# ruotianluo/ImageCaptioning.pytorch

Measured on NVIDIA H100. Metric: captions/sec at beam=5 seq_len=20, higher is better.
Workload: dtype f32 (fp32-grade: split-fp16 x3 tensor-core passes, fp32 accumulate)

## Files before the change

### imagecaptioning.pytorch_b200/_lib.py

```python
from __future__ import annotations

import ctypes
import os
from ctypes import POINTER, Structure, c_char_p, c_double, c_float, c_int, c_long, c_longlong, c_ulonglong, c_void_p

PKG = os.path.dirname(os.path.abspath(__file__))
LIB_PATH = os.path.join(PKG, 'libcapb200.so')

MODE_SIMT_FP32, MODE_TC_F16X3, MODE_TC_F16X1 = 0, 1, 2
MODES = {'simt_fp32': MODE_SIMT_FP32, 'tc_f16x3': MODE_TC_F16X3, 'tc_f16x1': MODE_TC_F16X1}
OP_MODES = dict(MODES, skinny_tf32x3=3, skinny_fp32=4, tf32x3_tc=5, tf32x3_tc_dgrad=6, tf32x3_tc_wgrad=7)
FAMILY_UPDOWN, FAMILY_NEWFC, FAMILY_ATT2IN2 = 0, 1, 2
FAMILY_AOA = 3
ENSEMBLE_MAX_MEMBERS = 8
SAMPLE_GREEDY, SAMPLE_MULTINOMIAL, SAMPLE_FORCED, SAMPLE_TEACHER, SAMPLE_TOPK, SAMPLE_TOPP = 0, 1, 2, 3, 4, 5


class ModelCfg(Structure):
    _fields_ = [('family', c_int), ('vocab_size', c_int), ('input_encoding_size', c_int), ('rnn_size', c_int), ('att_hid_size', c_int),
                ('fc_feat_size', c_int), ('att_feat_size', c_int), ('seq_length', c_int), ('numeric_mode', c_int)]


WEIGHT_FIELDS = ['embed', 'fc_embed_w', 'fc_embed_b', 'att_embed_w', 'att_embed_b', 'ctx2att_w', 'ctx2att_b', 'logit_w', 'logit_b',
                 'att_lstm_w_ih', 'att_lstm_w_hh', 'att_lstm_b_ih', 'att_lstm_b_hh', 'lang_lstm_w_ih', 'lang_lstm_w_hh', 'lang_lstm_b_ih',
# ... 162 lines not shown
                                        'logit_b')]


class GemmEpilogue(Structure):
    _fields_ = [('bias', c_void_p), ('row_bias', c_void_p), ('ld_row_bias', c_long), ('rows_per_group', c_int), ('residual', c_void_p),
                ('ld_res', c_long), ('relu', c_int), ('C', c_void_p), ('ldc', c_long), ('C_hi', c_void_p), ('C_lo', c_void_p), ('ldcs', c_long),
                ('lstm', c_int), ('H', c_int), ('c_prev', c_void_p), ('ld_cprev', c_long), ('src_row', c_void_p), ('c_out', c_void_p),
                ('ld_cout', c_long), ('gather_bias', c_void_p), ('ld_gb', c_long), ('gather_idx', c_void_p), ('h_f', c_void_p), ('h_hi', c_void_p),
                ('h_lo', c_void_p), ('ld_h', c_long)]


SIGNATURES = {
    'capb200_last_error': (c_char_p, []),
    'capb200_abi_version': (c_int, []),
    'capb200_range_status': (c_int, [c_int]),
    'capb200_linear': (c_int, [c_void_p, c_long, c_void_p, c_long, c_void_p, c_void_p, c_long, c_int, c_int, c_int, c_int, c_int, c_void_p]),
    'capb200_bench_linear': (c_int, [c_void_p, c_void_p, c_void_p, c_void_p, c_int, c_int, c_int, c_int, c_int, c_void_p, c_void_p]),
    'capb200_gemm_tile_n': (c_int, [c_int, c_int]),
    'capb200_gemm_tile_m': (c_int, [c_int, c_int]),
    'capb200_lstm_cell': (c_int, [c_void_p, c_int, c_void_p, c_void_p, c_void_p, c_void_p, c_void_p, c_void_p, c_void_p, c_void_p, c_int, c_int,
                                  c_int, c_void_p]),
    'capb200_additive_attention': (c_int, [c_void_p, c_void_p, c_void_p, c_void_p, c_void_p, c_void_p, c_void_p, c_int, c_int, c_int, c_int, c_int,
                                           c_void_p]),
    'capb200_log_softmax_topk': (c_int, [c_void_p, c_long, c_int, c_int, c_int, c_int, c_void_p, c_void_p, c_void_p]),
    'capb200_vocab_stats_topk': (c_int, [c_void_p, c_long, c_int, c_int, c_int, c_int, c_void_p, c_void_p, c_void_p, c_void_p]),
    'capb200_vocab_select': (c_int, [c_void_p, c_long, c_int, c_int, c_int, c_float, c_float, c_ulonglong, c_ulonglong, c_void_p, c_int, c_void_p,
                                     c_void_p, c_void_p]),
    'capb200_engine_create': (c_void_p, [POINTER(ModelCfg)]),
    'capb200_engine_destroy': (None, [c_void_p]),
    'capb200_engine_bind_weights': (c_int, [c_void_p, POINTER(Weights), c_void_p]),
    'capb200_engine_set_logit_layers': (c_int, [c_void_p, c_int]),
    'capb200_engine_bind_logit_head': (c_int, [c_void_p, POINTER(c_void_p), POINTER(c_void_p), c_void_p]),
    'capb200_engine_bind_logit_head_grads': (c_int, [c_void_p, POINTER(c_void_p), POINTER(c_void_p)]),
    'capb200_engine_set_logit_dropout': (c_int, [c_void_p, c_float]),
    'capb200_decode_beam': (c_int, [c_void_p, c_void_p, c_void_p, c_void_p, c_int, c_int, POINTER(BeamOpts), c_void_p, c_void_p, c_void_p, c_void_p,
                                    c_void_p, c_void_p, c_void_p]),
    'capb200_decode_beam_form': (c_int, [c_int, c_void_p, c_void_p, c_void_p, c_void_p, c_int, c_int, POINTER(BeamOpts), c_void_p, c_void_p, c_void_p,
                                         c_void_p, c_void_p, c_void_p, c_void_p]),
    'capb200_beam_record_logprobs': (c_int, [c_void_p, c_int, c_int, c_void_p, c_void_p]),
    'capb200_decode_beam_diverse': (c_int, [c_void_p, c_void_p, c_void_p, c_void_p, c_int, c_int, POINTER(DiverseOpts), c_void_p, c_void_p, c_void_p,
                                            c_void_p, c_void_p, c_void_p, c_void_p]),
    'capb200_decode_sample': (c_int, [c_void_p, c_void_p, c_void_p, c_void_p, c_int, c_int, POINTER(SampleOpts), c_void_p, c_long, c_void_p, c_void_p,
                                      c_void_p, c_void_p]),
    'capb200_engine_launch_count': (c_long, [c_void_p]),
    'capb200_engine_set_profiling': (c_int, [c_void_p, c_int]),
    'capb200_engine_read_profile': (c_int, [c_void_p, c_int, c_void_p, c_void_p, c_void_p, c_int]),
# ... 159 lines not shown
```

### imagecaptioning.pytorch_b200/csrc/engine.cu

```cuda
#include <map>
#include <mutex>
#include <vector>

#include "../../include/capb200.h"
#include "common.cuh"
#include "kernels.cuh"
#include "engine_common.cuh"
#include "train_common.cuh"

namespace capb200 {

static thread_local std::string g_last_error;
void set_error(const std::string& msg) { g_last_error = msg; }
const char* last_error_cstr() { return g_last_error.c_str(); }

__global__ void capb_fill_int_kernel(int* p, int n, int v) {
    const int i = blockIdx.x * blockDim.x + threadIdx.x;
    if (i < n) p[i] = v;
}
__global__ void capb_load_token_column_kernel(const long long* src, long ld, int col, int n, int* dst) {
    const int i = blockIdx.x * blockDim.x + threadIdx.x;
    if (i < n) dst[i] = (int)src[(long)i * ld + col];
}
__global__ void capb_store_token_column_kernel(const int* src, int n, long long* dst, long ld, int col) {
// ... 277 lines not shown
                g.epi.lstm = 1; g.epi.H = H;
                g.epi.c_prev = e->c0[cur]; g.epi.ld_cprev = e->ld_c; g.epi.src_row = src_row;
                g.epi.c_out = e->c0[nxt]; g.epi.ld_cout = e->ld_c;
                g.epi.gather_bias = xg ? e->xgate : nullptr; g.epi.ld_gb = e->ld_xgate; g.epi.gather_idx = tokens;
                g.epi.h_f = e->h0_out.v.f; g.epi.h_hi = e->h0_out.v.hi; g.epi.h_lo = e->h0_out.v.lo; g.epi.ld_h = e->h0_out.v.ld;
            } else {
                g.epi.C = e->gates.v.f; g.epi.ldc = e->gates.v.ld;
            }
            if (run_gemm(e, G_LSTM1, g, e->capRows, st)) return 1;
        }
        if (!e->tc) {
            e->launches++;
            if (lstm_pointwise_launch(rows, H, e->gates.v.f, e->gates.v.ld, src_row, e->c0[cur], e->ld_c, e->c0[nxt], e->ld_c, e->h0_out.v,
                                      xg ? e->xgate : nullptr, e->ld_xgate, tokens, st)) return 1;
        }
        {
            GemmProblem g;
            g.M = rows; g.N = A; g.nseg = 1;
            g.seg[0] = seg_of(e->h0_out.v, w.h2att_w, H, e->p_h2att, H);
            g.epi.bias = w.h2att_b;
            g.epi.C = e->att_h.v.f; g.epi.ldc = e->att_h.v.ld;
            if (run_gemm(e, G_H2ATT, g, e->capRows, st)) return 1;
        }
        e->launches += 2;
        if (additive_attention_launch(n_images, rpi, R, A, H, e->att_h.v.f, e->att_h.v.ld, e->p_att.v.f, e->p_att.v.ld, e->att_e.v.f, e->att_e.v.ld,
                                      mask, R, w.alpha_w, w.alpha_b, e->att_score, e->att_res.v, st)) return 1;
        {
            GemmProblem g;
            g.M = rows; g.N = 4 * H; g.nseg = 3;
            g.seg[0] = seg_of(e->att_res.v, w.lang_lstm_w_ih, 2 * H, e->p_l_ih_a, H);
            g.seg[1] = seg_of(e->h0_out.v, w.lang_lstm_w_ih + H, 2 * H, e->p_l_ih_h, H);
            g.seg[2] = seg_of(e->h1_in.v, w.lang_lstm_w_hh, H, e->p_l_hh, H);
            if (e->tc) {
                g.epi.bias = e->bsum_lang_il;
                g.epi.lstm = 1; g.epi.H = H;
                g.epi.c_prev = e->c1[cur]; g.epi.ld_cprev = e->ld_c; g.epi.src_row = src_row;
                g.epi.c_out = e->c1[nxt]; g.epi.ld_cout = e->ld_c;
                g.epi.h_f = e->h1_out.v.f; g.epi.h_hi = e->h1_out.v.hi; g.epi.h_lo = e->h1_out.v.lo; g.epi.ld_h = e->h1_out.v.ld;
            } else {
                g.epi.bias = e->bsum_lang;
                g.epi.C = e->gates.v.f; g.epi.ldc = e->gates.v.ld;
            }
            if (run_gemm(e, G_LSTM2, g, e->capRows, st)) return 1;
        }
        if (!e->tc) {
            e->launches++;
            if (lstm_pointwise_launch(rows, H, e->gates.v.f, e->gates.v.ld, src_row, e->c1[cur], e->ld_c, e->c1[nxt], e->ld_c, e->h1_out.v,
                                      nullptr, 0, nullptr, st)) return 1;
        }
        e->core_cur = nxt;
        return logit_gemm(e, e->h1_out.v, rows, logits, ld_logits, st);
    }
    if (e->cfg.family == CAPB200_FAMILY_ATT2IN2) {
        StateCopy s0, s1;
        s0.src = e->h0_out.v.f; s0.ld_src = e->h0_out.v.ld; s0.dst = e->h0_in.v;
        e->launches++;
        if (state_gather_embed_launch(rows, tokens, src_row, w.embed, E, E, 1, e->xt.v, H, 1, s0, s1, st)) return 1;
        const int cur = e->core_cur, nxt = cur ^ 1;
        {
            GemmProblem g;
            g.M = rows; g.N = A; g.nseg = 1;
            g.seg[0] = seg_of(e->h0_in.v, w.h2att_w, H, e->p_h2att, H);
            g.epi.bias = w.h2att_b;
            g.epi.C = e->att_h.v.f; g.epi.ldc = e->att_h.v.ld;
            if (run_gemm(e, G_H2ATT, g, e->capRows, st)) return 1;
        }
        e->launches += 2;
        if (additive_attention_launch(n_images, rpi, R, A, H, e->att_h.v.f, e->att_h.v.ld, e->p_att.v.f, e->p_att.v.ld, e->att_e.v.f, e->att_e.v.ld,
                                      mask, R, w.alpha_w, w.alpha_b, e->att_score, e->att_res.v, st)) return 1;
        {
            GemmProblem g;
            g.M = rows; g.N = 5 * H; g.nseg = 2;
            g.seg[0] = seg_of(e->xt.v, w.i2h_w, E, e->p_i2h, E);
            g.seg[1] = seg_of(e->h0_in.v, w.h2h_w, H, e->p_h2h, H);
            g.epi.bias = e->bsum_core;
            g.epi.C = e->gates.v.f; g.epi.ldc = e->gates.v.ld;
            if (run_gemm(e, G_CORE, g, e->capRows, st)) return 1;
        }
        {
            GemmProblem g;
            g.M = rows; g.N = 2 * H; g.nseg = 1;
            g.seg[0] = seg_of(e->att_res.v, w.a2c_w, H, e->p_a2c, H);
            g.epi.residual = e->gates.v.f + 3 * H; g.epi.ld_res = e->gates.v.ld;
            g.epi.C = e->gates.v.f + 3 * H; g.epi.ldc = e->gates.v.ld;
            if (run_gemm(e, G_A2C, g, e->capRows, st)) return 1;
        }
        e->launches++;
        if (maxout_pointwise_launch(rows, H, e->gates.v.f, e->gates.v.ld, src_row, e->c0[cur], e->ld_c, e->c0[nxt], e->ld_c, e->h0_out.v, st)) return 1;
        e->core_cur = nxt;
        return logit_gemm(e, e->h0_out.v, rows, logits, ld_logits, st);
// ... 459 lines not shown
                      const float* b_hh, float* h_out, float* c_out, int M, int H, int mode, void* stream) {
    cudaStream_t st = static_cast<cudaStream_t>(stream);
    CAPB_REQUIRE(x && h && c && w_ih && w_hh && b_ih && b_hh && h_out && c_out, "null argument");
    float* gates = nullptr;
    CAPB_CHECK_CUDA(cudaMallocAsync(&gates, sizeof(float) * ((size_t)M * 4 * H + 4 * H), st));
    float* bsum = gates + (size_t)M * 4 * H;
    add_vec_kernel<<<cdiv(4 * H, 256), 256, 0, st>>>(b_ih, b_hh, bsum, 4 * H);
    int rc = capb200_linear(x, Kx, w_ih, Kx, bsum, gates, 4 * H, M, 4 * H, Kx, 0, mode, stream);
    float* g2 = nullptr;
    if (!rc) {
        CAPB_CHECK_CUDA(cudaMallocAsync(&g2, sizeof(float) * (size_t)M * 4 * H, st));
        rc = capb200_linear(h, H, w_hh, H, nullptr, g2, 4 * H, M, 4 * H, H, 0, mode, stream);
        if (!rc) add_vec_kernel<<<cdiv(M * 4 * H, 256), 256, 0, st>>>(gates, g2, gates, M * 4 * H);
    }
    if (!rc) {
        ActView ho; ho.f = h_out; ho.ld = H;
        rc = lstm_pointwise_launch(M, H, gates, 4 * H, nullptr, c, H, c_out, H, ho, nullptr, 0, nullptr, st);
    }
    if (g2) cudaFreeAsync(g2, st);
    cudaFreeAsync(gates, st);
    return rc;
}

int capb200_additive_attention(const float* att_h, const float* p_att, const float* att, const float* mask, const float* alpha_w,
                               const float* alpha_b, float* out, int n_images, int rows_per_image, int R, int A, int H, void* stream) {
    CAPB_REQUIRE(att_h && p_att && att && alpha_w && alpha_b && out, "null argument");
    ActView o; o.f = out; o.ld = H;
    cudaStream_t st = static_cast<cudaStream_t>(stream);
    float* scratch = nullptr;
    CAPB_CHECK_CUDA(cudaMallocAsync(&scratch, sizeof(float) * (size_t)n_images * rows_per_image * R, st));
    const int rc = additive_attention_launch(n_images, rows_per_image, R, A, H, att_h, A, p_att, A, att, H, mask, R, alpha_w, alpha_b, scratch, o, st);
    cudaFreeAsync(scratch, st);
    return rc;
}

int capb200_log_softmax_topk(float* logits, long ld, int rows, int V1, int twice, int k, float* top_val, int* top_idx, void* stream) {
    CAPB_REQUIRE(logits != nullptr && rows > 0 && V1 > 0, "bad argument");
    VocabStepArgs va;
    va.rows = rows; va.V1 = V1; va.logits = logits; va.ld = ld; va.twice = twice; va.topk = k; va.top_val = top_val; va.top_idx = top_idx;
    return vocab_step_launch(va, static_cast<cudaStream_t>(stream));
}

int capb200_vocab_stats_topk(const float* logits, long ld, int rows, int V1, int twice, int k, float* stats, float* top_val, int* top_idx, void* stream) {
    CAPB_REQUIRE(logits != nullptr && stats != nullptr && top_val != nullptr && top_idx != nullptr, "null argument");
    CAPB_REQUIRE(rows > 0 && V1 > 0 && ld >= V1 && k > 0, "bad argument");
    CAPB_REQUIRE((reinterpret_cast<uintptr_t>(stats) & 7) == 0, "stats must be 8-byte aligned");
    VocabStepArgs va;
    va.rows = rows; va.V1 = V1; va.logits = const_cast<float*>(logits); va.ld = ld; va.twice = twice;
    va.topk = k; va.top_val = top_val; va.top_idx = top_idx;
    va.stats = reinterpret_cast<float2*>(stats);
    return vocab_step_launch(va, static_cast<cudaStream_t>(stream));
}

int capb200_vocab_select(float* logits, long ld, int rows, int V1, int select, float top, float temperature, unsigned long long seed,
                         unsigned long long step, int* unfinished, int first_step, int* tokens_out, float* picked_lp, void* stream) {
    CAPB_REQUIRE(logits != nullptr && tokens_out != nullptr && picked_lp != nullptr, "null argument");
// ... 745 lines not shown
```

### imagecaptioning.pytorch_b200/csrc/kernels.cuh

```cuda
#pragma once
#include "common.cuh"

namespace capb200 {

struct ActView {
    float* f = nullptr;
    __half* hi = nullptr;
    __half* lo = nullptr;
    long ld = 0;
};

struct StateCopy {
    const float* src = nullptr;
    long ld_src = 0;
    ActView dst;
};

__device__ __forceinline__ void copy_states4(long r, int src, int c4, int nstate, const StateCopy& sc0, const StateCopy& sc1) {
    float4 v0 = make_float4(0.f, 0.f, 0.f, 0.f), v1 = v0;
    if (src >= 0) {
        v0 = *reinterpret_cast<const float4*>(sc0.src + (long)src * sc0.ld_src + 4 * c4);
        if (nstate > 1) v1 = *reinterpret_cast<const float4*>(sc1.src + (long)src * sc1.ld_src + 4 * c4);
    }
    for (int s = 0; s < nstate; ++s) {
// ... 2 lines not shown
        *reinterpret_cast<float4*>(o.f + r * o.ld + 4 * c4) = v;
        if (o.hi != nullptr) {
            __align__(8) __half h[4];
            __align__(8) __half l[4];
            split_f32(v.x, h[0], l[0]); split_f32(v.y, h[1], l[1]); split_f32(v.z, h[2], l[2]); split_f32(v.w, h[3], l[3]);
            *reinterpret_cast<uint2*>(o.hi + r * o.ld + 4 * c4) = *reinterpret_cast<const uint2*>(h);
            *reinterpret_cast<uint2*>(o.lo + r * o.ld + 4 * c4) = *reinterpret_cast<const uint2*>(l);
        }
    }
}

int state_gather_embed_launch(int rows, const int* tokens, const int* src_row, const float* emb, long ld_emb, int E, int relu,
                              ActView xt, int H, int nstate, StateCopy sc0, StateCopy sc1, cudaStream_t stream);
int lstm_pointwise_launch(int rows, int H, const float* gates, long ld_g, const int* src_row, const float* c_prev, long ld_cp,
                          float* c_out, long ld_co, ActView h_out, const float* gather_bias, long ld_gb, const int* gather_idx,
                          cudaStream_t stream);
int relu_copy_launch(const float* x, long n, ActView out_flat, cudaStream_t stream);
int lstm_ln_launch(int rows, int H, const float* gates, long ld_g, const float* c_prev, long ld_cp, float* c_out, long ld_co, float* h_out, long ld_h,
                   const float* ln_a, const float* ln_b, float eps, float* ln_out, long ld_ln, cudaStream_t stream);
int maxout_pointwise_launch(int rows, int H, const float* sums, long ld_s, const int* src_row, const float* c_prev, long ld_cp,
                            float* c_out, long ld_co, ActView h_out, cudaStream_t stream);
int additive_attention_launch(int n_images, int rpi, int R, int A, int H, const float* att_h, long ld_ah, const float* p_att, long ld_pa,
                              const float* att, long ld_at, const float* mask, long ld_mask, const float* alpha_w, const float* alpha_b,
                              float* score_scratch , ActView out, cudaStream_t stream, float* alpha_out = nullptr );
int mask_rows_launch(ActView x, int n_images, int R, int cols, const float* mask, long ld_mask, cudaStream_t stream);
int ss_select_launch(int rows, int V1, const float* prev_logp, long ld, const long long* labels, long ld_labels, int col, unsigned long long seed, float prob,
                     int* tok_out, cudaStream_t stream);

struct DecodeEdits {
    int constraint = 0;
    int unk_col = -1;
    int n_bad = 0;
    const int* bad = nullptr;
    int trigrams = 0;
    int trigram_rows = 0;
    __host__ __device__ bool any() const { return constraint != 0 || unk_col >= 0 || n_bad > 0 || trigrams != 0; }
    __host__ __device__ int kinds() const { return (constraint ? 1 : 0) + (unk_col >= 0 ? 1 : 0) + (n_bad > 0 ? 1 : 0); }
};

struct VocabStepArgs {
    int rows = 0;
    int V1 = 0;
    float* logits = nullptr;
    long ld = 0;
    int twice = 0;
    float2* stats = nullptr;
    int topk = 0;
// ... 221 lines not shown
```

### imagecaptioning.pytorch_b200/csrc/pointwise.cu

```cuda
#include "common.cuh"
#include "kernels.cuh"

namespace capb200 {

static int pw_blocks(long total) {
    long b = (total + 255) / 256;
    return (int)(b > sm_count() * 8 ? sm_count() * 8 : b);
}

namespace {

__device__ __forceinline__ float sigmoidf_(float x) { return fast_sigmoid(x); }

__device__ __forceinline__ void store_act(const ActView& o, long row, int col, float v) {
    o.f[row * o.ld + col] = v;
    if (o.hi != nullptr) {
        __half h, l;
        split_f32(v, h, l);
        o.hi[row * o.ld + col] = h;
        o.lo[row * o.ld + col] = l;
    }
}

__global__ void state_gather_embed_kernel(int rows, const int* __restrict__ tokens, const int* __restrict__ src_row,
// ... 84 lines not shown
#pragma unroll
    for (int u = 0; u < 8; ++u) { const int c = threadIdx.x + 256 * u; if (c < H) ln_out[(long)r * ld_ln + c] = __ldg(ln_a + c) * (hv[u] - mean) * inv + __ldg(ln_b + c); }
}

__global__ void maxout_pointwise_kernel(int rows, int H, const float* __restrict__ sums, long ld_s, const int* __restrict__ src_row,
                                        const float* __restrict__ c_prev, long ld_cp, float* __restrict__ c_out, long ld_co, ActView h_out) {
    const long total = (long)rows * H;
    for (long i = blockIdx.x * (long)blockDim.x + threadIdx.x; i < total; i += (long)gridDim.x * blockDim.x) {
        const int r = (int)(i / H), c = (int)(i % H);
        const float* s = sums + (long)r * ld_s;
        const float gi = sigmoidf_(s[c]), gf = sigmoidf_(s[H + c]), go = sigmoidf_(s[2 * H + c]);
        const float gg = fmaxf(s[3 * H + c], s[4 * H + c]);
        const int src = src_row ? src_row[r] : r;
        const float cp = (src < 0 || c_prev == nullptr) ? 0.f : c_prev[(long)src * ld_cp + c];
        const float cn = gf * cp + gi * gg;
        const float hn = go * fast_tanh(cn);
        c_out[(long)r * ld_co + c] = cn;
        store_act(h_out, r, c, hn);
    }
}

constexpr int ATT_JB = 5;
constexpr int ATT_SW = 8;
template <int NA>
__global__ void __launch_bounds__(ATT_SW * 32, NA <= 16 ? 5 : 2) att_score_kernel(int rpi, int R, int A, const float* __restrict__ att_h, long ld_ah,
                                                                const float* __restrict__ p_att, long ld_pa, const float* __restrict__ alpha_w,
                                                                const float* __restrict__ alpha_b_ptr, float* __restrict__ score) {
    extern __shared__ float s_ah[];
    constexpr int AP = NA * 32;
    float* s_w = s_ah + ATT_JB * AP;
    constexpr float kC = 2.885390081777927f;
    const int img = blockIdx.y;
    const int warp = threadIdx.x >> 5, lane = threadIdx.x & 31;
    const int r = blockIdx.x * ATT_SW + warp;
    const float alpha_b = __ldg(alpha_b_ptr);
    float pv[NA];
    const bool live = r < R;
    const float* pr = p_att + ((long)img * R + (live ? r : 0)) * ld_pa;
    for (int i = threadIdx.x; i < AP; i += ATT_SW * 32) s_w[i] = (i < A) ? __ldg(alpha_w + i) : 0.f;
    __syncthreads();
    float wsum = 0.f;
#pragma unroll
    for (int k = 0; k < NA; ++k) {
        const int a = (NA % 4 == 0) ? 128 * (k >> 2) + 4 * lane + (k & 3) : lane + 32 * k;
        pv[k] = (live && a < A) ? __ldg(pr + a) * kC : 0.f;
        wsum += s_w[a];
    }
    for (int j0 = 0; j0 < rpi; j0 += ATT_JB) {
        const int nj = min(ATT_JB, rpi - j0);
        __syncthreads();
        for (int i = threadIdx.x; i < nj * AP; i += ATT_SW * 32) {
            const int j = i / AP, a = i - j * AP;
            s_ah[i] = (a < A) ? att_h[((long)img * rpi + j0 + j) * ld_ah + a] * kC : 0.f;
        }
        __syncthreads();
        if (live) {
            float part[ATT_JB];
#pragma unroll
            for (int j = 0; j < ATT_JB; ++j) {
                part[j] = 0.f;
                if (j < nj) {
                    if (NA % 4 == 0) {
                        float acc = 0.f;
#pragma unroll
                        for (int g = 0; g < NA / 4; ++g) {
                            const float4 ah = *reinterpret_cast<const float4*>(&s_ah[j * AP + 128 * g + 4 * lane]);
                            const float z[4] = {pv[4 * g] + ah.x, pv[4 * g + 1] + ah.y, pv[4 * g + 2] + ah.z, pv[4 * g + 3] + ah.w};
                            float y[4];
#pragma unroll
                            for (int u = 0; u < 4; ++u) {
                                float e;
                                asm("ex2.approx.ftz.f32 %0, %1;" : "=f"(e) : "f"(fminf(z[u], 28.0f)));
                                y[u] = 1.0f + e;
                            }
                            const float p01 = y[0] * y[1], p23 = y[2] * y[3];
                            float rr;
                            asm("rcp.approx.ftz.f32 %0, %1;" : "=f"(rr) : "f"(p01 * p23));
                            const float r01 = rr * p23, r23 = rr * p01;
                            const float4 w4 = *reinterpret_cast<const float4*>(&s_w[128 * g + 4 * lane]);
                            acc = fmaf(w4.x, r01 * y[1], acc);
                            acc = fmaf(w4.y, r01 * y[0], acc);
                            acc = fmaf(w4.z, r23 * y[3], acc);
                            acc = fmaf(w4.w, r23 * y[2], acc);
                        }
                        part[j] = fmaf(-2.0f, acc, wsum);
                    } else {
#pragma unroll
                        for (int k = 0; k < NA; ++k) {
                            float e;
                            asm("ex2.approx.ftz.f32 %0, %1;" : "=f"(e) : "f"(fminf(pv[k] + s_ah[j * AP + lane + 32 * k], 28.0f)));
                            part[j] = fmaf(s_w[lane + 32 * k], 1.0f - __fdividef(2.0f, 1.0f + e), part[j]);
                        }
                    }
                }
            }
#pragma unroll
            for (int j = 0; j < ATT_JB; ++j) {
                float v = part[j];
#pragma unroll
                for (int o = 16; o > 0; o >>= 1) v += __shfl_xor_sync(0xffffffffu, v, o);
                if (lane == 0 && j < nj) score[((long)img * rpi + j0 + j) * R + r] = v + alpha_b;
            }
        }
    }
}

constexpr int ATT_CT = 256;
__global__ void __launch_bounds__(ATT_CT) att_combine_kernel(int rpi, int R, int H, const float* __restrict__ score, const float* __restrict__ att,
                                                             long ld_at, const float* __restrict__ mask, long ld_mask, ActView out,
                                                             float* __restrict__ alpha_out) {
    extern __shared__ float s_w[];
    const int img = blockIdx.x;
    const int c = blockIdx.y * ATT_CT + threadIdx.x;
    const int warp = threadIdx.x >> 5, lane = threadIdx.x & 31;
    for (int j0 = 0; j0 < rpi; j0 += ATT_JB) {
        const int nj = min(ATT_JB, rpi - j0);
        __syncthreads();
        if (warp < nj) {
            const float* sc = score + ((long)img * rpi + j0 + warp) * R;
            float* w = s_w + warp * R;
            float mx = -INFINITY;
            for (int r = lane; r < R; r += 32) mx = fmaxf(mx, sc[r]);
#pragma unroll
            for (int o = 16; o > 0; o >>= 1) mx = fmaxf(mx, __shfl_xor_sync(0xffffffffu, mx, o));
            float sum = 0.f;
            for (int r = lane; r < R; r += 32) { const float e = expf(sc[r] - mx); w[r] = e; sum += e; }
#pragma unroll
            for (int o = 16; o > 0; o >>= 1) sum += __shfl_xor_sync(0xffffffffu, sum, o);
            const float inv = 1.0f / sum;
            float msum = 0.f;
            for (int r = lane; r < R; r += 32) {
                float v = w[r] * inv;
                if (mask != nullptr) { v *= mask[(long)img * ld_mask + r]; msum += v; }
                w[r] = v;
            }
            if (mask != nullptr) {
#pragma unroll
                for (int o = 16; o > 0; o >>= 1) msum += __shfl_xor_sync(0xffffffffu, msum, o);
                for (int r = lane; r < R; r += 32) w[r] = w[r] / msum;
            }
        }
        __syncthreads();
        if (alpha_out != nullptr && blockIdx.y == 0) {
            for (int i = threadIdx.x; i < nj * R; i += ATT_CT) alpha_out[((long)img * rpi + j0) * R + i] = s_w[i];
        }
        if (c < H) {
            float acc[ATT_JB];
#pragma unroll
            for (int j = 0; j < ATT_JB; ++j) acc[j] = 0.f;
            const float* ap = att + (long)img * R * ld_at + c;
            for (int r = 0; r < R; ++r) {
                const float v = __ldg(ap + (long)r * ld_at);
#pragma unroll
                for (int j = 0; j < ATT_JB; ++j)
                    if (j < nj) acc[j] = fmaf(s_w[j * R + r], v, acc[j]);
            }
#pragma unroll
            for (int j = 0; j < ATT_JB; ++j)
                if (j < nj) store_act(out, (long)img * rpi + j0 + j, c, acc[j]);
        }
    }
}

__global__ void relu_copy_kernel(const float* __restrict__ x, long n, ActView out_flat) {
    for (long i = blockIdx.x * (long)blockDim.x + threadIdx.x; i < n; i += (long)gridDim.x * blockDim.x) {
        const float v = fmaxf(__ldg(x + i), 0.f);
        out_flat.f[i] = v;
        if (out_flat.hi) { __half h, l; split_f32(v, h, l); out_flat.hi[i] = h; out_flat.lo[i] = l; }
    }
}

}

int relu_copy_launch(const float* x, long n, ActView out_flat, cudaStream_t stream) {
    relu_copy_kernel<<<pw_blocks(n), 256, 0, stream>>>(x, n, out_flat);
    CAPB_CHECK_CUDA(cudaGetLastError());
    return 0;
}

int state_gather_embed_launch(int rows, const int* tokens, const int* src_row, const float* emb, long ld_emb, int E, int relu,
                              ActView xt, int H, int nstate, StateCopy sc0, StateCopy sc1, cudaStream_t stream) {
    if (rows <= 0) return 0;
    state_gather_embed_kernel<<<rows, 256, 0, stream>>>(rows, tokens, src_row, emb, ld_emb, E, relu, xt, H, nstate, sc0, sc1);
// ... 9 lines not shown
    lstm_pointwise_kernel<<<pw_blocks((long)rows * H), 256, 0, stream>>>(rows, H, gates, ld_g, src_row, c_prev, ld_cp, c_out, ld_co, h_out,
                                                                          gather_bias, ld_gb, gather_idx);
    CAPB_CHECK_CUDA(cudaGetLastError());
    return 0;
}

int lstm_ln_launch(int rows, int H, const float* gates, long ld_g, const float* c_prev, long ld_cp, float* c_out, long ld_co, float* h_out, long ld_h,
                   const float* ln_a, const float* ln_b, float eps, float* ln_out, long ld_ln, cudaStream_t stream) {
    if (rows <= 0) return 0;
    CAPB_REQUIRE(H <= 2048, "lstm_ln: hidden size above 2048");
    lstm_ln_kernel<<<rows, 256, 0, stream>>>(H, gates, ld_g, c_prev, ld_cp, c_out, ld_co, h_out, ld_h, ln_a, ln_b, eps, ln_out, ld_ln);
    CAPB_CHECK_CUDA(cudaGetLastError());
    return 0;
}

int maxout_pointwise_launch(int rows, int H, const float* sums, long ld_s, const int* src_row, const float* c_prev, long ld_cp,
                            float* c_out, long ld_co, ActView h_out, cudaStream_t stream) {
    if (rows <= 0) return 0;
    maxout_pointwise_kernel<<<pw_blocks((long)rows * H), 256, 0, stream>>>(rows, H, sums, ld_s, src_row, c_prev, ld_cp, c_out, ld_co, h_out);
    CAPB_CHECK_CUDA(cudaGetLastError());
    return 0;
}

int additive_attention_launch(int n_images, int rpi, int R, int A, int H, const float* att_h, long ld_ah, const float* p_att, long ld_pa,
                              const float* att, long ld_at, const float* mask, long ld_mask, const float* alpha_w, const float* alpha_b,
                              float* score_scratch, ActView out, cudaStream_t stream, float* alpha_out) {
    if (n_images <= 0 || rpi <= 0) return 0;
    CAPB_REQUIRE(A <= 1024, "attention: att_hid_size above 1024");
    CAPB_REQUIRE(score_scratch != nullptr, "attention: score scratch missing");
    const int na = cdiv(A, 32);
    dim3 sgrid(cdiv(R, ATT_SW), n_images);
#define CAPB_ATT_CASE(NA_)                                                                                                             \
    att_score_kernel<NA_><<<sgrid, ATT_SW * 32, sizeof(float) * (ATT_JB + 1) * NA_ * 32, stream>>>(rpi, R, A, att_h, ld_ah, p_att, ld_pa, alpha_w, \
                                                                                               alpha_b, score_scratch)
    if (na <= 2) CAPB_ATT_CASE(2);
    else if (na <= 4) CAPB_ATT_CASE(4);
    else if (na <= 8) CAPB_ATT_CASE(8);
    else if (na <= 16) CAPB_ATT_CASE(16);
    else CAPB_ATT_CASE(32);
#undef CAPB_ATT_CASE
    CAPB_CHECK_CUDA(cudaGetLastError());
    const size_t smem = sizeof(float) * (size_t)ATT_JB * R;
    CAPB_REQUIRE(smem <= 48 * 1024, "attention: too many regions");
    dim3 grid(n_images, cdiv(H, ATT_CT));
    att_combine_kernel<<<grid, ATT_CT, smem, stream>>>(rpi, R, H, score_scratch, att, ld_at, mask, ld_mask, out, alpha_out);
    CAPB_CHECK_CUDA(cudaGetLastError());
    return 0;
}

}
```

### include/capb200.h

```cpp
#ifndef CAPB200_H_
#define CAPB200_H_

#ifdef __cplusplus
extern "C" {
#endif

#define CAPB200_ABI_VERSION 1

#define CAPB200_MODE_SIMT_FP32 0
#define CAPB200_MODE_TC_F16X3 1
#define CAPB200_MODE_TC_F16X1 2
#define CAPB200_MODE_SKINNY_TF32X3 3
#define CAPB200_MODE_SKINNY_FP32 4
#define CAPB200_MODE_TF32X3_TC 5
#define CAPB200_MODE_TF32X3_TC_DGRAD 6
#define CAPB200_MODE_TF32X3_TC_WGRAD 7

#define CAPB200_MAX_SEQ_LENGTH 256

#define CAPB200_FAMILY_UPDOWN 0
#define CAPB200_FAMILY_NEWFC 1
#define CAPB200_FAMILY_ATT2IN2 2

typedef struct capb200_engine capb200_engine;
typedef struct capb200_cider_table capb200_cider_table;

const char* capb200_last_error(void);
int capb200_abi_version(void);
int capb200_range_status(int reset);


int capb200_linear(const float* x, long ldx, const float* w, long ldw, const float* b, float* y, long ldy, int M, int N, int K,
                   int relu, int mode, void* stream);

int capb200_bench_linear(const float* x, const float* w, const float* b, float* y, int M, int N, int K, int mode, int iters, float* ms_per_launch,
                         void* stream);

int capb200_gemm_tile_n(int M, int N);
int capb200_gemm_tile_m(int M, int N);

int capb200_lstm_cell(const float* x, int Kx, const float* h, const float* c, const float* w_ih, const float* w_hh, const float* b_ih,
                      const float* b_hh, float* h_out, float* c_out, int M, int H, int mode, void* stream);

int capb200_additive_attention(const float* att_h, const float* p_att, const float* att, const float* mask, const float* alpha_w,
                               const float* alpha_b, float* out, int n_images, int rows_per_image, int R, int A, int H, void* stream);

int capb200_log_softmax_topk(float* logits, long ld, int rows, int V1, int twice, int k, float* top_val, int* top_idx, void* stream);

int capb200_vocab_stats_topk(const float* logits, long ld, int rows, int V1, int twice, int k, float* stats, float* top_val, int* top_idx,
                             void* stream);

int capb200_vocab_select(float* logits, long ld, int rows, int V1, int select, float top, float temperature, unsigned long long seed,
                         unsigned long long step, int* unfinished, int first_step, int* tokens_out, float* picked_lp, void* stream);

typedef struct {
    int family;
    int vocab_size;
    int input_encoding_size;
    int rnn_size;
    int att_hid_size;
    int fc_feat_size;
    int att_feat_size;
    int seq_length;
    int numeric_mode;
} capb200_model_cfg;

typedef struct {
    const float* embed;
// ... 501 lines not shown
```

Before: 24630.

## Fuse attention score, softmax and weighted combine into one per-image kernel

Adds a single-launch attention kernel that runs one block per image and computes region scores, the masked softmax in shared memory, and the weighted context combine, with an L2 bulk prefetch of the region features. It becomes the default whenever attention weights are not requested, replacing the two-kernel score/combine path and its global score scratch round-trip. In exchange, parallelism drops to one 512-thread block per image, so small batches may underuse the GPU compared with the previous multi-block grids.

```diff
diff --git a/imagecaptioning.pytorch_b200/_lib.py b/imagecaptioning.pytorch_b200/_lib.py
--- a/imagecaptioning.pytorch_b200/_lib.py
+++ b/imagecaptioning.pytorch_b200/_lib.py
@@ -208,6 +208,8 @@
                                   c_int, c_void_p]),
     'capb200_additive_attention': (c_int, [c_void_p, c_void_p, c_void_p, c_void_p, c_void_p, c_void_p, c_void_p, c_int, c_int, c_int, c_int, c_int,
                                            c_void_p]),
+    'capb200_additive_attention_form': (c_int, [c_int, c_void_p, c_void_p, c_void_p, c_void_p, c_void_p, c_void_p, c_void_p, c_void_p, c_void_p, c_int,
+                                                c_int, c_int, c_int, c_int, c_void_p]),
     'capb200_log_softmax_topk': (c_int, [c_void_p, c_long, c_int, c_int, c_int, c_int, c_void_p, c_void_p, c_void_p]),
     'capb200_vocab_stats_topk': (c_int, [c_void_p, c_long, c_int, c_int, c_int, c_int, c_void_p, c_void_p, c_void_p, c_void_p]),
     'capb200_vocab_select': (c_int, [c_void_p, c_long, c_int, c_int, c_int, c_float, c_float, c_ulonglong, c_ulonglong, c_void_p, c_int, c_void_p,
diff --git a/imagecaptioning.pytorch_b200/csrc/engine.cu b/imagecaptioning.pytorch_b200/csrc/engine.cu
--- a/imagecaptioning.pytorch_b200/csrc/engine.cu
+++ b/imagecaptioning.pytorch_b200/csrc/engine.cu
@@ -323,7 +323,7 @@
             g.epi.C = e->att_h.v.f; g.epi.ldc = e->att_h.v.ld;
             if (run_gemm(e, G_H2ATT, g, e->capRows, st)) return 1;
         }
-        e->launches += 2;
+        e->launches++;
         if (additive_attention_launch(n_images, rpi, R, A, H, e->att_h.v.f, e->att_h.v.ld, e->p_att.v.f, e->p_att.v.ld, e->att_e.v.f, e->att_e.v.ld,
                                       mask, R, w.alpha_w, w.alpha_b, e->att_score, e->att_res.v, st)) return 1;
         {
@@ -366,7 +366,7 @@
             g.epi.C = e->att_h.v.f; g.epi.ldc = e->att_h.v.ld;
             if (run_gemm(e, G_H2ATT, g, e->capRows, st)) return 1;
         }
-        e->launches += 2;
+        e->launches++;
         if (additive_attention_launch(n_images, rpi, R, A, H, e->att_h.v.f, e->att_h.v.ld, e->p_att.v.f, e->p_att.v.ld, e->att_e.v.f, e->att_e.v.ld,
                                       mask, R, w.alpha_w, w.alpha_b, e->att_score, e->att_res.v, st)) return 1;
         {
@@ -872,16 +872,25 @@
     return rc;
 }
 
-int capb200_additive_attention(const float* att_h, const float* p_att, const float* att, const float* mask, const float* alpha_w,
-                               const float* alpha_b, float* out, int n_images, int rows_per_image, int R, int A, int H, void* stream) {
+int capb200_additive_attention_form(int form, const float* att_h, const float* p_att, const float* att, const float* mask, const float* alpha_w,
+                                    const float* alpha_b, float* out, void* out_hi, void* out_lo, int n_images, int rows_per_image, int R, int A,
+                                    int H, void* stream) {
     CAPB_REQUIRE(att_h && p_att && att && alpha_w && alpha_b && out, "null argument");
-    ActView o; o.f = out; o.ld = H;
+    CAPB_REQUIRE((out_hi == nullptr) == (out_lo == nullptr), "out_hi and out_lo come together");
+    ActView o; o.f = out; o.ld = H; o.hi = static_cast<__half*>(out_hi); o.lo = static_cast<__half*>(out_lo);
     cudaStream_t st = static_cast<cudaStream_t>(stream);
     float* scratch = nullptr;
     CAPB_CHECK_CUDA(cudaMallocAsync(&scratch, sizeof(float) * (size_t)n_images * rows_per_image * R, st));
-    const int rc = additive_attention_launch(n_images, rows_per_image, R, A, H, att_h, A, p_att, A, att, H, mask, R, alpha_w, alpha_b, scratch, o, st);
+    const int rc = additive_attention_launch(n_images, rows_per_image, R, A, H, att_h, A, p_att, A, att, H, mask, R, alpha_w, alpha_b, scratch, o, st,
+                                             nullptr, form);
     cudaFreeAsync(scratch, st);
     return rc;
+}
+
+int capb200_additive_attention(const float* att_h, const float* p_att, const float* att, const float* mask, const float* alpha_w,
+                               const float* alpha_b, float* out, int n_images, int rows_per_image, int R, int A, int H, void* stream) {
+    return capb200_additive_attention_form(0, att_h, p_att, att, mask, alpha_w, alpha_b, out, nullptr, nullptr, n_images, rows_per_image, R, A, H,
+                                           stream);
 }
 
 int capb200_log_softmax_topk(float* logits, long ld, int rows, int V1, int twice, int k, float* top_val, int* top_idx, void* stream) {
diff --git a/imagecaptioning.pytorch_b200/csrc/kernels.cuh b/imagecaptioning.pytorch_b200/csrc/kernels.cuh
--- a/imagecaptioning.pytorch_b200/csrc/kernels.cuh
+++ b/imagecaptioning.pytorch_b200/csrc/kernels.cuh
@@ -48,7 +48,8 @@
                             float* c_out, long ld_co, ActView h_out, cudaStream_t stream);
 int additive_attention_launch(int n_images, int rpi, int R, int A, int H, const float* att_h, long ld_ah, const float* p_att, long ld_pa,
                               const float* att, long ld_at, const float* mask, long ld_mask, const float* alpha_w, const float* alpha_b,
-                              float* score_scratch , ActView out, cudaStream_t stream, float* alpha_out = nullptr );
+                              float* score_scratch , ActView out, cudaStream_t stream, float* alpha_out = nullptr ,
+                              int form = 0);
 int mask_rows_launch(ActView x, int n_images, int R, int cols, const float* mask, long ld_mask, cudaStream_t stream);
 int ss_select_launch(int rows, int V1, const float* prev_logp, long ld, const long long* labels, long ld_labels, int col, unsigned long long seed, float prob,
                      int* tok_out, cudaStream_t stream);
diff --git a/imagecaptioning.pytorch_b200/csrc/pointwise.cu b/imagecaptioning.pytorch_b200/csrc/pointwise.cu
--- a/imagecaptioning.pytorch_b200/csrc/pointwise.cu
+++ b/imagecaptioning.pytorch_b200/csrc/pointwise.cu
@@ -130,6 +130,141 @@
 
 constexpr int ATT_JB = 5;
 constexpr int ATT_SW = 8;
+constexpr int ATT_CT = 256;
+constexpr int ATT_FT = 512;
+constexpr int ATT_NC = 2;
+constexpr int ATT_RB = 4;
+
+constexpr float ATT_KC = 2.885390081777927f;
+
+template <int NA>
+__device__ __forceinline__ float att_load_region(const float* __restrict__ pr, bool live, int A, int lane, const float* s_w, float (&pv)[NA]) {
+    float wsum = 0.f;
+#pragma unroll
+    for (int k = 0; k < NA; ++k) {
+        const int a = (NA % 4 == 0) ? 128 * (k >> 2) + 4 * lane + (k & 3) : lane + 32 * k;
+        pv[k] = (live && a < A) ? __fmul_rn(__ldg(pr + a), ATT_KC) : 0.f;
+        wsum += s_w[a];
+    }
+    return wsum;
+}
+
+template <int NA>
+__device__ __forceinline__ void att_score_rows(const float (&pv)[NA], const float* s_ah, const float* s_w, float wsum, int nj, int lane,
+                                               float (&part)[ATT_JB]) {
+    constexpr int AP = NA * 32;
+#pragma unroll
+    for (int j = 0; j < ATT_JB; ++j) {
+        part[j] = 0.f;
+        if (j < nj) {
+            if (NA % 4 == 0) {
+                float acc = 0.f;
+#pragma unroll
+                for (int g = 0; g < NA / 4; ++g) {
+                    const float4 ah = *reinterpret_cast<const float4*>(&s_ah[j * AP + 128 * g + 4 * lane]);
+                    const float z[4] = {pv[4 * g] + ah.x, pv[4 * g + 1] + ah.y, pv[4 * g + 2] + ah.z, pv[4 * g + 3] + ah.w};
+                    float y[4];
+#pragma unroll
+                    for (int u = 0; u < 4; ++u) {
+                        float e;
+                        asm("ex2.approx.ftz.f32 %0, %1;" : "=f"(e) : "f"(fminf(z[u], 28.0f)));
+                        y[u] = 1.0f + e;
+                    }
+                    const float p01 = y[0] * y[1], p23 = y[2] * y[3];
+                    float rr;
+                    asm("rcp.approx.ftz.f32 %0, %1;" : "=f"(rr) : "f"(p01 * p23));
+                    const float r01 = rr * p23, r23 = rr * p01;
+                    const float4 w4 = *reinterpret_cast<const float4*>(&s_w[128 * g + 4 * lane]);
+                    acc = fmaf(w4.x, r01 * y[1], acc);
+                    acc = fmaf(w4.y, r01 * y[0], acc);
+                    acc = fmaf(w4.z, r23 * y[3], acc);
+                    acc = fmaf(w4.w, r23 * y[2], acc);
+                }
+                part[j] = fmaf(-2.0f, acc, wsum);
+            } else {
+#pragma unroll
+                for (int k = 0; k < NA; ++k) {
+                    float e;
+                    asm("ex2.approx.ftz.f32 %0, %1;" : "=f"(e) : "f"(fminf(pv[k] + s_ah[j * AP + lane + 32 * k], 28.0f)));
+                    part[j] = fmaf(s_w[lane + 32 * k], 1.0f - __fdividef(2.0f, 1.0f + e), part[j]);
+                }
+            }
+        }
+    }
+#pragma unroll
+    for (int j = 0; j < ATT_JB; ++j) {
+#pragma unroll
+        for (int o = 16; o > 0; o >>= 1) part[j] += __shfl_xor_sync(0xffffffffu, part[j], o);
+    }
+}
+
+__device__ __forceinline__ void att_softmax_row(const float* sc, float* w, int R, const float* __restrict__ mask_row, int lane) {
+    float mx = -INFINITY;
+    for (int r = lane; r < R; r += 32) mx = fmaxf(mx, sc[r]);
+#pragma unroll
+    for (int o = 16; o > 0; o >>= 1) mx = fmaxf(mx, __shfl_xor_sync(0xffffffffu, mx, o));
+    float sum = 0.f;
+    for (int r = lane; r < R; r += 32) { const float e = expf(sc[r] - mx); w[r] = e; sum += e; }
+#pragma unroll
+    for (int o = 16; o > 0; o >>= 1) sum += __shfl_xor_sync(0xffffffffu, sum, o);
+    const float inv = 1.0f / sum;
+    float msum = 0.f;
+    for (int r = lane; r < R; r += 32) {
+        float v = w[r] * inv;
+        if (mask_row != nullptr) { v *= mask_row[r]; msum += v; }
+        w[r] = v;
+    }
+    if (mask_row != nullptr) {
+#pragma unroll
+        for (int o = 16; o > 0; o >>= 1) msum += __shfl_xor_sync(0xffffffffu, msum, o);
+        for (int r = lane; r < R; r += 32) w[r] = w[r] / msum;
+    }
+}
+
+template <int NC, int RB>
+__device__ __forceinline__ void att_combine_columns(const float* __restrict__ att_img, long ld_at, int R, const float* s_w, int nj, int c, int stride,
+                                                    int H, const ActView& out, long row0) {
+    float acc[NC][ATT_JB];
+    bool in[NC];
+#pragma unroll
+    for (int q = 0; q < NC; ++q) {
+        in[q] = c + q * stride < H;
+#pragma unroll
+        for (int j = 0; j < ATT_JB; ++j) acc[q][j] = 0.f;
+    }
+    int r = 0;
+    for (; r + RB <= R; r += RB) {
+        float v[RB][NC];
+#pragma unroll
+        for (int u = 0; u < RB; ++u)
+#pragma unroll
+            for (int q = 0; q < NC; ++q) v[u][q] = in[q] ? __ldg(att_img + (long)(r + u) * ld_at + c + q * stride) : 0.f;
+#pragma unroll
+        for (int u = 0; u < RB; ++u)
+#pragma unroll
+            for (int j = 0; j < ATT_JB; ++j)
+                if (j < nj) {
+                    const float a = s_w[j * R + r + u];
+#pragma unroll
+                    for (int q = 0; q < NC; ++q) acc[q][j] = fmaf(a, v[u][q], acc[q][j]);
+                }
+    }
+    for (; r < R; ++r) {
+#pragma unroll
+        for (int q = 0; q < NC; ++q) {
+            const float v = in[q] ? __ldg(att_img + (long)r * ld_at + c + q * stride) : 0.f;
+#pragma unroll
+            for (int j = 0; j < ATT_JB; ++j)
+                if (j < nj) acc[q][j] = fmaf(s_w[j * R + r], v, acc[q][j]);
+        }
+    }
+#pragma unroll
+    for (int q = 0; q < NC; ++q)
+#pragma unroll
+        for (int j = 0; j < ATT_JB; ++j)
+            if (in[q] && j < nj) store_act(out, row0 + j, c + q * stride, acc[q][j]);
+}
+
 template <int NA>
 __global__ void __launch_bounds__(ATT_SW * 32, NA <= 16 ? 5 : 2) att_score_kernel(int rpi, int R, int A, const float* __restrict__ att_h, long ld_ah,
                                                                 const float* __restrict__ p_att, long ld_pa, const float* __restrict__ alpha_w,
@@ -137,7 +272,6 @@
     extern __shared__ float s_ah[];
     constexpr int AP = NA * 32;
     float* s_w = s_ah + ATT_JB * AP;
-    constexpr float kC = 2.885390081777927f;
     const int img = blockIdx.y;
     const int warp = threadIdx.x >> 5, lane = threadIdx.x & 31;
     const int r = blockIdx.x * ATT_SW + warp;
@@ -147,73 +281,25 @@
     const float* pr = p_att + ((long)img * R + (live ? r : 0)) * ld_pa;
     for (int i = threadIdx.x; i < AP; i += ATT_SW * 32) s_w[i] = (i < A) ? __ldg(alpha_w + i) : 0.f;
     __syncthreads();
-    float wsum = 0.f;
-#pragma unroll
-    for (int k = 0; k < NA; ++k) {
-        const int a = (NA % 4 == 0) ? 128 * (k >> 2) + 4 * lane + (k & 3) : lane + 32 * k;
-        pv[k] = (live && a < A) ? __ldg(pr + a) * kC : 0.f;
-        wsum += s_w[a];
-    }
+    const float wsum = att_load_region<NA>(pr, live, A, lane, s_w, pv);
     for (int j0 = 0; j0 < rpi; j0 += ATT_JB) {
         const int nj = min(ATT_JB, rpi - j0);
         __syncthreads();
         for (int i = threadIdx.x; i < nj * AP; i += ATT_SW * 32) {
             const int j = i / AP, a = i - j * AP;
-            s_ah[i] = (a < A) ? att_h[((long)img * rpi + j0 + j) * ld_ah + a] * kC : 0.f;
+            s_ah[i] = (a < A) ? att_h[((long)img * rpi + j0 + j) * ld_ah + a] * ATT_KC : 0.f;
         }
         __syncthreads();
         if (live) {
             float part[ATT_JB];
-#pragma unroll
-            for (int j = 0; j < ATT_JB; ++j) {
-                part[j] = 0.f;
-                if (j < nj) {
-                    if (NA % 4 == 0) {
-                        float acc = 0.f;
-#pragma unroll
-                        for (int g = 0; g < NA / 4; ++g) {
-                            const float4 ah = *reinterpret_cast<const float4*>(&s_ah[j * AP + 128 * g + 4 * lane]);
-                            const float z[4] = {pv[4 * g] + ah.x, pv[4 * g + 1] + ah.y, pv[4 * g + 2] + ah.z, pv[4 * g + 3] + ah.w};
-                            float y[4];
-#pragma unroll
-                            for (int u = 0; u < 4; ++u) {
-                                float e;
-                                asm("ex2.approx.ftz.f32 %0, %1;" : "=f"(e) : "f"(fminf(z[u], 28.0f)));
-                                y[u] = 1.0f + e;
-                            }
-                            const float p01 = y[0] * y[1], p23 = y[2] * y[3];
-                            float rr;
-                            asm("rcp.approx.ftz.f32 %0, %1;" : "=f"(rr) : "f"(p01 * p23));
-                            const float r01 = rr * p23, r23 = rr * p01;
-                            const float4 w4 = *reinterpret_cast<const float4*>(&s_w[128 * g + 4 * lane]);
-                            acc = fmaf(w4.x, r01 * y[1], acc);
-                            acc = fmaf(w4.y, r01 * y[0], acc);
-                            acc = fmaf(w4.z, r23 * y[3], acc);
-                            acc = fmaf(w4.w, r23 * y[2], acc);
-                        }
-                        part[j] = fmaf(-2.0f, acc, wsum);
-                    } else {
-#pragma unroll
-                        for (int k = 0; k < NA; ++k) {
-                            float e;
-                            asm("ex2.approx.ftz.f32 %0, %1;" : "=f"(e) : "f"(fminf(pv[k] + s_ah[j * AP + lane + 32 * k], 28.0f)));
-                            part[j] = fmaf(s_w[lane + 32 * k], 1.0f - __fdividef(2.0f, 1.0f + e), part[j]);
-                        }
-                    }
-                }
-            }
-#pragma unroll
-            for (int j = 0; j < ATT_JB; ++j) {
-                float v = part[j];
-#pragma unroll
-                for (int o = 16; o > 0; o >>= 1) v += __shfl_xor_sync(0xffffffffu, v, o);
-                if (lane == 0 && j < nj) score[((long)img * rpi + j0 + j) * R + r] = v + alpha_b;
-            }
-        }
-    }
-}
-
-constexpr int ATT_CT = 256;
+            att_score_rows<NA>(pv, s_ah, s_w, wsum, nj, lane, part);
+#pragma unroll
+            for (int j = 0; j < ATT_JB; ++j)
+                if (lane == 0 && j < nj) score[((long)img * rpi + j0 + j) * R + r] = part[j] + alpha_b;
+        }
+    }
+}
+
 __global__ void __launch_bounds__(ATT_CT) att_combine_kernel(int rpi, int R, int H, const float* __restrict__ score, const float* __restrict__ att,
                                                              long ld_at, const float* __restrict__ mask, long ld_mask, ActView out,
                                                              float* __restrict__ alpha_out) {
@@ -224,49 +310,68 @@
     for (int j0 = 0; j0 < rpi; j0 += ATT_JB) {
         const int nj = min(ATT_JB, rpi - j0);
         __syncthreads();
-        if (warp < nj) {
-            const float* sc = score + ((long)img * rpi + j0 + warp) * R;
-            float* w = s_w + warp * R;
-            float mx = -INFINITY;
-            for (int r = lane; r < R; r += 32) mx = fmaxf(mx, sc[r]);
-#pragma unroll
-            for (int o = 16; o > 0; o >>= 1) mx = fmaxf(mx, __shfl_xor_sync(0xffffffffu, mx, o));
-            float sum = 0.f;
-            for (int r = lane; r < R; r += 32) { const float e = expf(sc[r] - mx); w[r] = e; sum += e; }
-#pragma unroll
-            for (int o = 16; o > 0; o >>= 1) sum += __shfl_xor_sync(0xffffffffu, sum, o);
-            const float inv = 1.0f / sum;
-            float msum = 0.f;
-            for (int r = lane; r < R; r += 32) {
-                float v = w[r] * inv;
-                if (mask != nullptr) { v *= mask[(long)img * ld_mask + r]; msum += v; }
-                w[r] = v;
-            }
-            if (mask != nullptr) {
-#pragma unroll
-                for (int o = 16; o > 0; o >>= 1) msum += __shfl_xor_sync(0xffffffffu, msum, o);
-                for (int r = lane; r < R; r += 32) w[r] = w[r] / msum;
-            }
-        }
+        if (warp < nj)
+            att_softmax_row(score + ((long)img * rpi + j0 + warp) * R, s_w + warp * R, R, mask != nullptr ? mask + (long)img * ld_mask : nullptr, lane);
         __syncthreads();
         if (alpha_out != nullptr && blockIdx.y == 0) {
             for (int i = threadIdx.x; i < nj * R; i += ATT_CT) alpha_out[((long)img * rpi + j0) * R + i] = s_w[i];
         }
-        if (c < H) {
-            float acc[ATT_JB];
-#pragma unroll
-            for (int j = 0; j < ATT_JB; ++j) acc[j] = 0.f;
-            const float* ap = att + (long)img * R * ld_at + c;
-            for (int r = 0; r < R; ++r) {
-                const float v = __ldg(ap + (long)r * ld_at);
-#pragma unroll
-                for (int j = 0; j < ATT_JB; ++j)
-                    if (j < nj) acc[j] = fmaf(s_w[j * R + r], v, acc[j]);
+        if (c < H) att_combine_columns<1, 1>(att + (long)img * R * ld_at, ld_at, R, s_w, nj, c, ATT_CT, H, out, (long)img * rpi + j0);
+    }
+}
+
+template <int NA>
+__global__ void __launch_bounds__(ATT_FT, NA <= 16 ? 2 : 1) att_fused_kernel(int rpi, int R, int A, int H, const float* __restrict__ att_h, long ld_ah,
+                                                                             const float* __restrict__ p_att, long ld_pa, const float* __restrict__ att,
+                                                                             long ld_at, const float* __restrict__ alpha_w,
+                                                                             const float* __restrict__ alpha_b_ptr, const float* __restrict__ mask,
+                                                                             long ld_mask, ActView out) {
+    extern __shared__ float s_ah[];
+    constexpr int AP = NA * 32;
+    constexpr int NW = ATT_FT / 32;
+    float* s_w = s_ah + ATT_JB * AP;
+    float* s_sc = s_w + AP;
+    const int img = blockIdx.x;
+    const int warp = threadIdx.x >> 5, lane = threadIdx.x & 31;
+    const float* pa_img = p_att + (long)img * R * ld_pa;
+    const float* at_img = att + (long)img * R * ld_at;
+    if (warp == 0) {
+        auto prefetch = [&](const float* base, long ld, int cols) {
+            if (((reinterpret_cast<uintptr_t>(base) | (uintptr_t)(ld * 4)) & 15) != 0) return;
+            const long bytes = (((long)(R - 1) * ld + cols) * 4) & ~15L;
+            for (long off = (long)lane * 16384; off < bytes; off += 32L * 16384) {
+                const unsigned n = (unsigned)min(16384L, bytes - off);
+                asm volatile("cp.async.bulk.prefetch.L2.global [%0], %1;" ::"l"(reinterpret_cast<const char*>(base) + off), "r"(n) : "memory");
             }
+        };
+        prefetch(pa_img, ld_pa, A);
+        prefetch(at_img, ld_at, H);
+    }
+    const float alpha_b = __ldg(alpha_b_ptr);
+    for (int i = threadIdx.x; i < AP; i += ATT_FT) s_w[i] = (i < A) ? __ldg(alpha_w + i) : 0.f;
+    const float* mask_row = mask != nullptr ? mask + (long)img * ld_mask : nullptr;
+    for (int j0 = 0; j0 < rpi; j0 += ATT_JB) {
+        const int nj = min(ATT_JB, rpi - j0);
+        __syncthreads();
+        for (int i = threadIdx.x; i < nj * AP; i += ATT_FT) {
+            const int j = i / AP, a = i - j * AP;
+            s_ah[i] = (a < A) ? att_h[((long)img * rpi + j0 + j) * ld_ah + a] * ATT_KC : 0.f;
+        }
+        __syncthreads();
+        for (int r = warp; r < R; r += NW) {
+            float pv[NA];
+            const float wsum = att_load_region<NA>(pa_img + (long)r * ld_pa, true, A, lane, s_w, pv);
+            float part[ATT_JB];
+            att_score_rows<NA>(pv, s_ah, s_w, wsum, nj, lane, part);
 #pragma unroll
             for (int j = 0; j < ATT_JB; ++j)
-                if (j < nj) store_act(out, (long)img * rpi + j0 + j, c, acc[j]);
-        }
+                if (lane == 0 && j < nj) s_sc[j * R + r] = part[j] + alpha_b;
+        }
+        __syncthreads();
+        if (warp < nj) att_softmax_row(s_sc + warp * R, s_sc + warp * R, R, mask_row, lane);
+        __syncthreads();
+        for (int c = threadIdx.x; c < H; c += ATT_NC * ATT_FT)
+            att_combine_columns<ATT_NC, ATT_RB>(at_img, ld_at, R, s_sc, nj, c, ATT_FT, H, out, (long)img * rpi + j0);
     }
 }
 
@@ -322,13 +427,42 @@
     return 0;
 }
 
+static size_t att_weights_smem(int R) { return sizeof(float) * (size_t)ATT_JB * R; }
+
+template <int NA>
+static int att_fused_launch(int n_images, int rpi, int R, int A, int H, const float* att_h, long ld_ah, const float* p_att, long ld_pa,
+                             const float* att, long ld_at, const float* mask, long ld_mask, const float* alpha_w, const float* alpha_b, ActView out,
+                             cudaStream_t stream) {
+    constexpr size_t kFixed = sizeof(float) * (ATT_JB + 1) * NA * 32;
+    static bool attr_set = false;
+    if (!attr_set) {
+        CAPB_CHECK_CUDA(cudaFuncSetAttribute(att_fused_kernel<NA>, cudaFuncAttributeMaxDynamicSharedMemorySize, (int)(kFixed + 48 * 1024)));
+        attr_set = true;
+    }
+    att_fused_kernel<NA><<<n_images, ATT_FT, kFixed + att_weights_smem(R), stream>>>(rpi, R, A, H, att_h, ld_ah, p_att, ld_pa, att, ld_at, alpha_w,
+                                                                                    alpha_b, mask, ld_mask, out);
+    return 0;
+}
+
 int additive_attention_launch(int n_images, int rpi, int R, int A, int H, const float* att_h, long ld_ah, const float* p_att, long ld_pa,
                               const float* att, long ld_at, const float* mask, long ld_mask, const float* alpha_w, const float* alpha_b,
-                              float* score_scratch, ActView out, cudaStream_t stream, float* alpha_out) {
+                              float* score_scratch, ActView out, cudaStream_t stream, float* alpha_out, int form) {
     if (n_images <= 0 || rpi <= 0) return 0;
     CAPB_REQUIRE(A <= 1024, "attention: att_hid_size above 1024");
+    CAPB_REQUIRE(att_weights_smem(R) <= 48 * 1024, "attention: too many regions");
+    CAPB_REQUIRE(form >= 0 && form <= 2, "attention: form is 0, 1 or 2");
+    const bool fused = form == 0 ? alpha_out == nullptr : form == 2;
+    CAPB_REQUIRE(!fused || alpha_out == nullptr, "attention: the one-launch form does not write the attention weights");
+    const int na = cdiv(A, 32);
+    if (fused) {
+#define CAPB_ATT_CASE(NA_) att_fused_launch<NA_>(n_images, rpi, R, A, H, att_h, ld_ah, p_att, ld_pa, att, ld_at, mask, ld_mask, alpha_w, alpha_b, out, stream)
+        const int rc = na <= 2 ? CAPB_ATT_CASE(2) : na <= 4 ? CAPB_ATT_CASE(4) : na <= 8 ? CAPB_ATT_CASE(8) : na <= 16 ? CAPB_ATT_CASE(16) : CAPB_ATT_CASE(32);
+#undef CAPB_ATT_CASE
+        if (rc) return rc;
+        CAPB_CHECK_CUDA(cudaGetLastError());
+        return 0;
+    }
     CAPB_REQUIRE(score_scratch != nullptr, "attention: score scratch missing");
-    const int na = cdiv(A, 32);
     dim3 sgrid(cdiv(R, ATT_SW), n_images);
 #define CAPB_ATT_CASE(NA_)                                                                                                             \
     att_score_kernel<NA_><<<sgrid, ATT_SW * 32, sizeof(float) * (ATT_JB + 1) * NA_ * 32, stream>>>(rpi, R, A, att_h, ld_ah, p_att, ld_pa, alpha_w, \
@@ -340,12 +474,10 @@
     else CAPB_ATT_CASE(32);
 #undef CAPB_ATT_CASE
     CAPB_CHECK_CUDA(cudaGetLastError());
-    const size_t smem = sizeof(float) * (size_t)ATT_JB * R;
-    CAPB_REQUIRE(smem <= 48 * 1024, "attention: too many regions");
     dim3 grid(n_images, cdiv(H, ATT_CT));
-    att_combine_kernel<<<grid, ATT_CT, smem, stream>>>(rpi, R, H, score_scratch, att, ld_at, mask, ld_mask, out, alpha_out);
-    CAPB_CHECK_CUDA(cudaGetLastError());
-    return 0;
-}
-
-}
+    att_combine_kernel<<<grid, ATT_CT, att_weights_smem(R), stream>>>(rpi, R, H, score_scratch, att, ld_at, mask, ld_mask, out, alpha_out);
+    CAPB_CHECK_CUDA(cudaGetLastError());
+    return 0;
+}
+
+}
diff --git a/include/capb200.h b/include/capb200.h
--- a/include/capb200.h
+++ b/include/capb200.h
@@ -44,6 +44,9 @@
 
 int capb200_additive_attention(const float* att_h, const float* p_att, const float* att, const float* mask, const float* alpha_w,
                                const float* alpha_b, float* out, int n_images, int rows_per_image, int R, int A, int H, void* stream);
+int capb200_additive_attention_form(int form, const float* att_h, const float* p_att, const float* att, const float* mask, const float* alpha_w,
+                                    const float* alpha_b, float* out, void* out_hi, void* out_lo, int n_images, int rows_per_image, int R, int A,
+                                    int H, void* stream);
 
 int capb200_log_softmax_topk(float* logits, long ld, int rows, int V1, int twice, int k, float* top_val, int* top_idx, void* stream);
 
```

After: 25000, median of 6. 1.5% higher.
